# tohtsky/myFM

Measured on AMD Instinct MI355X. Metric: Gibbs iterations/sec (rank=32), higher is better.
Workload: dtype f64

## Files before the change

### include/myfm_hip.h

```cpp
#ifndef MYFM_HIP_H_
#define MYFM_HIP_H_

#include <stdint.h>

#ifdef __cplusplus
extern "C" {
#endif

#define MFM_OK 0
#define MFM_ERR_INVALID 1
#define MFM_ERR_RUNTIME 2
#define MFM_ERR_DEVICE 3

#define MFM_TASK_REGRESSION 0
#define MFM_TASK_CLASSIFICATION 1
#define MFM_TASK_ORDERED 2

typedef struct mfm_ctx mfm_ctx;
typedef struct mfm_design mfm_design;
typedef struct mfm_store mfm_store;

const char *mfm_version(void);
int mfm_device_count(void);
const char *mfm_global_error(void);
// ... 20 lines not shown
int mfm_peer_drop(mfm_ctx *ctx);
int mfm_set_main_levels(mfm_ctx *ctx, const int32_t *level, int64_t D0);
int mfm_set_row_offset(mfm_ctx *ctx, int64_t first_global_row);

int mfm_set_main(mfm_ctx *ctx, int64_t N, int64_t D0, const int64_t *indptr, const int32_t *indices,
                 const double *data, const double *y);
int mfm_add_block(mfm_ctx *ctx, int64_t B, int64_t Db, const int64_t *indptr, const int32_t *indices,
                  const double *data, const int64_t *original_to_block);
int mfm_set_groups(mfm_ctx *ctx, const int32_t *group_index, int64_t D, int32_t G);
int mfm_set_residual_policy(mfm_ctx *ctx, int32_t recomputable);
int mfm_finalize(mfm_ctx *ctx, int32_t rank);

int64_t mfm_dim_all(const mfm_ctx *ctx);
int mfm_plan_info(const mfm_ctx *ctx, int64_t *n_levels_main, int64_t *n_launches_per_sweep);
int mfm_plan_flags(const mfm_ctx *ctx);
#define MFM_RES_INFO_FIELDS 15
int mfm_res_info(const mfm_ctx *ctx, int64_t *out, int n_out, char *why, int why_len);
#define MFM_CELL_INFO_FIELDS 74
int mfm_cell_info(const mfm_ctx *ctx, int64_t *out, int n_out, char *why, int why_len);

int mfm_set_state(mfm_ctx *ctx, double w0, const double *w, const double *V);
int mfm_get_state(mfm_ctx *ctx, double *w0, double *w, double *V);
int mfm_set_w0(mfm_ctx *ctx, double w0);
int mfm_zero_w(mfm_ctx *ctx);
int mfm_get_e(mfm_ctx *ctx, double *e);
int mfm_get_q(mfm_ctx *ctx, double *q);
int mfm_set_e(mfm_ctx *ctx, const double *e);

int mfm_reduce_e(mfm_ctx *ctx, double *sum_e, double *sum_e2);
int mfm_shift_e(mfm_ctx *ctx, double delta);
int mfm_group_stats_w(mfm_ctx *ctx, const double *mu_w, double *sum, double *ssd);
// ... 193 lines not shown
```

### myfm_amd/_build.py

```python
import os
import subprocess
import sys
import sysconfig

HERE = os.path.dirname(os.path.abspath(__file__))
ROOT = os.path.dirname(HERE)
CSRC = os.path.join(HERE, "csrc")
INCLUDE = os.path.join(ROOT, "include")
HIP_LIB = os.path.join(HERE, "libmyfm_hip.so")
EXT_SUFFIX = sysconfig.get_config_var("EXT_SUFFIX") or ".so"
PYMOD = os.path.join(HERE, "_myfm" + EXT_SUFFIX)

HIP_UNITS = {
    "mfm_hip.hip": ["mfm_env.hpp", "mfm_common.hpp", "mfm_wave.hpp", "mfm_policies.hpp", "mfm_kernels.hpp", "mfm_mf_kernels.hpp", "mfm_res.hpp", "mfm_res_plan.hpp",
                    "mfm_plan.hpp", "mfm_block_kernels.hpp", "mfm_erfcx.hpp", "mfm_tasks.hpp", "mfm_tn.hpp", "mfm_philox.hpp", "mfm_predict.hpp", "mfm_samples.hpp", "mfm_dist.hpp", "mfm_rng.hpp", "mfm_mtjump.hpp", "mfm_cell.hpp",
                    "mfm_chain_api.hpp", "mfm_rng_state.hpp", "mfm_latent_api.hpp", "mfm_latent_host.hpp", "mfm_comm.hpp"],
    "mfm_latent.hip": ["mfm_env.hpp", "mfm_common.hpp", "mfm_rng_state.hpp", "mfm_latent_api.hpp"],
    "mfm_cell.hip": ["mfm_env.hpp", "mfm_common.hpp", "mfm_wave.hpp", "mfm_cell.hpp"],
    "mfm_chain.hip": ["mfm_env.hpp", "mfm_common.hpp", "mfm_wave.hpp", "mfm_policies.hpp", "mfm_chain_api.hpp", "mfm_chain_plan.hpp", "mfm_chain_stream.hpp"],
    "mfm_vb.hip": ["mfm_env.hpp", "mfm_common.hpp", "mfm_erfcx.hpp", "mfm_vb.hpp", "mfm_comm.hpp"],
    "mfm_pairs.hip": ["mfm_env.hpp", "mfm_common.hpp", "mfm_pairs.hpp", "mfm_pairs_rank.hpp", "mfm_pairs_ucb.hpp", "mfm_samples.hpp"],
    "mfm_foldin.hip": ["mfm_env.hpp", "mfm_common.hpp", "mfm_foldin.hpp", "mfm_foldin_handle.hpp", "mfm_philox.hpp", "mfm_samples.hpp"],
    "mfm_foldin_gibbs.hip": ["mfm_env.hpp", "mfm_common.hpp", "mfm_foldin.hpp", "mfm_foldin_gibbs.hpp", "mfm_foldin_gibbs_plan.hpp",
                             "mfm_foldin_handle.hpp", "mfm_tn.hpp", "mfm_philox.hpp", "mfm_samples.hpp"],
}
OBJ_DIR = os.path.join(CSRC, "_obj")
PYMOD_HEADERS = ["mfm_env.hpp", "mfm_hostnormals.hpp", "mfm_mtjump.hpp"]


# ... 83 lines not shown
```

### myfm_amd/_capi.py

```python
import ctypes as C
import os

import numpy as np
import scipy.sparse as sps

_HERE = os.path.dirname(os.path.abspath(__file__))
LIB_PATH = os.path.join(_HERE, "libmyfm_hip.so")

MFM_OK, MFM_ERR_INVALID, MFM_ERR_RUNTIME, MFM_ERR_DEVICE = 0, 1, 2, 3
TASK_REGRESSION, TASK_CLASSIFICATION, TASK_ORDERED = 0, 1, 2

SYMBOLS = [
    "mfm_version", "mfm_device_count", "mfm_global_error", "mfm_create", "mfm_destroy", "mfm_last_error",
    "mfm_set_stream", "mfm_synchronize", "mfm_set_main", "mfm_add_block", "mfm_set_groups", "mfm_finalize",
    "mfm_peer_info", "mfm_peer_set", "mfm_peer_model_info", "mfm_peer_set_model", "mfm_peer_export", "mfm_peer_import", "mfm_peer_drop", "mfm_set_residual_policy", "mfm_dim_all", "mfm_plan_info", "mfm_plan_flags", "mfm_res_info", "mfm_cell_info", "mfm_set_state", "mfm_get_state", "mfm_set_w0", "mfm_zero_w", "mfm_get_e",
    "mfm_get_q", "mfm_set_e", "mfm_reduce_e", "mfm_shift_e", "mfm_group_stats_w", "mfm_group_stats_V",
    "mfm_sweep_w", "mfm_sweep_V", "mfm_sweep_wV", "mfm_update_e_regression", "mfm_update_e_classification", "mfm_score_train",
    "mfm_oprobit_add_group", "mfm_oprobit_eval", "mfm_oprobit_sample_z", "mfm_hyper_stats", "mfm_timing_enable", "mfm_timing_select", "mfm_timing_reset",
    "mfm_timing_n_classes", "mfm_timing_class_name", "mfm_timing_get", "mfm_design_create", "mfm_design_add_block",
    "mfm_design_destroy", "mfm_design_last_error", "mfm_design_dim_all", "mfm_design_predict",
    "mfm_host_column_levels", "mfm_rng_prepare", "mfm_rng_seed_mt19937", "mfm_rng_set_program", "mfm_rng_prefetch", "mfm_rng_acquire",
    "mfm_rng_get_z", "mfm_design_score_ctx", "mfm_design_n_rows", "mfm_set_allreduce", "mfm_set_row_offset", "mfm_set_main_levels",
    "mfm_test_erfcx", "mfm_test_truncated_normal", "mfm_get_device", "mfm_set_shard", "mfm_comm_unique_id", "mfm_comm_init",
    "mfm_comm_stats", "mfm_comm_info", "mfm_store_create", "mfm_store_destroy", "mfm_store_last_error", "mfm_store_size", "mfm_store_push_ctx",
# ... 424 lines not shown
        self._ck(lib().mfm_rng_host_read(self.h, int(offset), int(n), _p(out)))
        return out[: int(n)]

    def rng_host_advance(self, words):
        self._ck(lib().mfm_rng_host_advance(self.h, int(words)))

    def set_residual_policy(self, recomputable):
        self._ck(lib().mfm_set_residual_policy(self.h, 1 if recomputable else 0))

    def plan_flags(self):
        f = lib().mfm_plan_flags(self.h)
        return {"qfree": bool(f & 1), "unit": bool(f & 2), "ell": bool(f & 4), "sharded": bool(f & 8), "soa": bool(f & 16),
                "fused_next": bool(f & 32), "sharded_fused": bool(f & 64), "mf": bool(f & 128), "resident": bool(f & 256), "cell": bool(f & 512), "streamed_chain": bool(f & 1024), "resident_overflow": bool(f & 2048)}

    RES_INFO = ("ready", "G", "RV", "RL", "RX", "umax", "n_items", "item_bits", "n_runs", "max_wg_users", "max_slice_items",
                "e_where", "n_rows", "s2_in_sweep_b", "lds_bytes")
    E_WHERE = ("rows", "slots", "slots_with_sums", "cell", "dropped")

    def res_info(self):
        out = np.zeros(len(self.RES_INFO), dtype=np.int64)
        why = C.create_string_buffer(256)
        self._ck(lib().mfm_res_info(self.h, _p(out), out.shape[0], why, len(why)))
        d = dict(zip(self.RES_INFO, (int(v) for v in out)))
        d["ready"] = bool(d["ready"])
        d["e_where"] = self.E_WHERE[d["e_where"]]
        d["why"] = why.value.decode()
        return d

    CELL_INFO = ("ready", "G", "umax", "item32", "n_streams", "n_fields", "N", "Npad", "max_steps", "chunk_max", "chunk_min",
                 "chunks_empty", "split_mask", "score_fb")
    CELL_STREAM_TYPE = ("U", "I", "C")
# ... 416 lines not shown
```

### myfm_amd/csrc/_myfm.cpp

```cpp
#include <thread>
#include <cstdio>
#include <pybind11/functional.h>
#include <pybind11/numpy.h>
#include <pybind11/pybind11.h>
#include <pybind11/stl.h>

#include <algorithm>
#include <cmath>
#include <chrono>
#include <cstdint>
#include <cstdlib>
#include <functional>
#include <limits>
#include <memory>
#include <random>
#include <set>
#include <sstream>
#include <stdexcept>
#include <string>
#include <tuple>
#include <type_traits>
#include <vector>

#include "mfm_env.hpp"
// ... 2880 lines not shown
             char path[512];
             if (mfm_comm_info(s.trainer->ctx, &n, path, sizeof(path)) != MFM_OK) throw std::runtime_error(mfm_global_error());
             return py::make_tuple((int)n, std::string(path));
           },
           "(ranks of the library's own RCCL communicator (ncclCommCount), path of the librccl.so it bound); (0, '') without one")
      .def("step", &GibbsSession::step, py::call_guard<py::gil_scoped_release>())
      .def("synchronize", &GibbsSession::synchronize)
      .def("residual", &GibbsSession::residual)
      .def("timing_enable", &GibbsSession::timing_enable)
      .def("timing_select", &GibbsSession::timing_select)
      .def("timing_reset", &GibbsSession::timing_reset)
      .def("timing", &GibbsSession::timing)
      .def("plan_info", &GibbsSession::plan_info)
      .def("latent_info", &GibbsSession::latent_info)
      .def("plan_flags", [](GibbsSession &s) { return mfm_plan_flags(s.trainer->ctx); })
      .def("peer_info",
           [](GibbsSession &s) {
             int32_t pending = 0;
             void *sum = nullptr, *flag = nullptr;
             int64_t sb = 0, fb = 0;
             ck(s.trainer->ctx, mfm_peer_info(s.trainer->ctx, &pending, &sum, &flag, &sb, &fb));
             return py::make_tuple(pending != 0, (uintptr_t)sum, (uintptr_t)flag, sb, fb);
           })
      .def("peer_set",
           [](GibbsSession &s, int world, int rank, const std::vector<uintptr_t> &sums, const std::vector<uintptr_t> &flags) {
             if ((int)sums.size() != world || (int)flags.size() != world) throw std::invalid_argument("peer_set: one buffer pair per rank");
             std::vector<void *> a, b;
             for (auto v : sums) a.push_back((void *)v);
             for (auto v : flags) b.push_back((void *)v);
             ck(s.trainer->ctx, mfm_peer_set(s.trainer->ctx, world, rank, a.data(), b.data()));
// ... 143 lines not shown
```

### myfm_amd/csrc/mfm_hip.hip

```cpp
#include <algorithm>
#include <cerrno>
#include <chrono>
#include <cmath>
#include <cstdio>
#include <cstring>
#include <map>
#include <memory>
#include <mutex>
#include <string>
#include <thread>
#include <type_traits>
#include <vector>

#include <fcntl.h>
#include <sys/file.h>
#include <sys/stat.h>
#include <unistd.h>

#include <hipcub/hipcub.hpp>

#include "mfm_common.hpp"
#include "mfm_kernels.hpp"
#include "mfm_plan.hpp"
#include "mfm_res_plan.hpp"
// ... 1561 lines not shown
    case VPath::ShardedTwoField: form = 64 | 128; break;
    case VPath::Deferred:
    case VPath::Generic:
    case VPath::Cell:
      break;
  }
  return (streamed ? 1024 : 0) | (ctx->res.ready && ctx->res.RX > 0 ? 2048 : 0) | form | (ctx->X.unit ? 2 : 0) | (ctx->X.ell_width >= 0 ? 4 : 0) |
         (ctx->comm.active() ? 8 : 0) | (ctx->res.ready ? 256 : 0) | (ctx->cell.ready ? 512 : 0);
}

int mfm_res_info(const mfm_ctx *ctx, int64_t *out, int n_out, char *why, int why_len) {
  if (!ctx || n_out < 0 || (n_out > 0 && !out) || why_len < 0 || (why_len > 0 && !why)) return MFM_ERR_INVALID;
  const ResPlan &rp = ctx->res;
  const int64_t v[MFM_RES_INFO_FIELDS] = {rp.ready ? 1 : 0, rp.G,       rp.RV,     rp.RL,           rp.RX,
                                          rp.umax,          rp.n_items, rp.item_bits, rp.n_runs,    rp.max_wg_users,
                                          rp.max_slice_items, (int64_t)ctx->e_where, rp.n_rows, rp.s2b, (int64_t)rp.lds_bytes};
  for (int i = 0; i < n_out; i++) out[i] = i < MFM_RES_INFO_FIELDS ? v[i] : 0;
  if (why_len > 0) {
    std::strncpy(why, rp.ready ? "" : rp.why.c_str(), (size_t)why_len - 1);
    why[why_len - 1] = 0;
  }
  return MFM_OK;
}

int mfm_cell_info(const mfm_ctx *ctx, int64_t *out, int n_out, char *why, int why_len) {
  if (!ctx || n_out < 0 || (n_out > 0 && !out) || why_len < 0 || (why_len > 0 && !why)) return MFM_ERR_INVALID;
  const CellPlan &cp = ctx->cell;
  int64_t v[MFM_CELL_INFO_FIELDS] = {0};
  const int m = (int)cp.fields.size(), ns = (int)cp.streams.size();
  int64_t split = 0;
  const bool typed = ns > 0 && cp.sU == 0;
// ... 915 lines not shown
```

### myfm_amd/csrc/mfm_res.hpp

```cpp
#pragma once
#include <algorithm>
#include <cstdlib>
#include <cstring>
#include <atomic>
#include <string>
#include <thread>
#include <type_traits>
#include <vector>

#include "mfm_common.hpp"
#include "mfm_mf_kernels.hpp"

namespace mfm {

#ifndef MFM_RES_CH
#define MFM_RES_CH 4
#endif
constexpr int RES_MAX_PEERS = 8;

struct ResArgs {
  double2 *eq;
  const double *e_in;
  double *e_slots;
  const int32_t *perm;
  const uint32_t *uidw;
  const uint32_t *headw;
  const int32_t *run_item;
  const int32_t *first_run;
  const int32_t *wg_run_ptr;
  const int32_t *wg_nruns;
  const int32_t *wg_user_ptr;
  const int2 *user_desc;
  const int32_t *wg_item_ptr;
  const int32_t *ent_ptr;
  const int2 *entries;
  const int32_t *scols;
  const int2 *item_desc;
  double *partials;
  double *dv;
  double *V;
  int64_t D;
  int f_begin, f_end;
  int linear;
  int n_sw;
  double *w;
  const double *zw;
  const double *lam_w, *mu_w;
  double e_shift;
  const double *z;
  const double *lam, *mu;
// ... 4 lines not shown
  int n_items, umax;
  unsigned long long *bar;
  int n_wg;
  int *error;
  unsigned long long *prof;
  int xworld, xrank;
  unsigned long long xepoch0;
  double *xsum[RES_MAX_PEERS];
  unsigned long long *xflag[RES_MAX_PEERS];
  unsigned long long *xarrive;
  int xmodel;
  double *xw[RES_MAX_PEERS], *xV[RES_MAX_PEERS];
  int ngx;
  int no_store;
  int xch_break;
};

__device__ __forceinline__ void res_store2(double *p, double a, double b) {
  __hip_atomic_store(p, a, __ATOMIC_RELAXED, __HIP_MEMORY_SCOPE_AGENT);
  __hip_atomic_store(p + 1, b, __ATOMIC_RELAXED, __HIP_MEMORY_SCOPE_AGENT);
}

enum { RES_BAR_START = 0, RES_BAR_TOP = 16, RES_BAR_XCNT = 32, RES_BAR_GEN = 160, RES_BAR_CENSUS = 288, RES_BAR_WORDS = 416 };
struct ResBar {
  int xcc;
  unsigned long long n_x, nx;
};

__device__ __forceinline__ bool res_spin(const ResArgs &a, const unsigned long long *w, unsigned long long target, bool &dead) {
  unsigned spins = 0;
// ... 125 lines not shown
#define RES_STAMP0(k) \
  if (a.prof && tid == 0) a.prof[(int64_t)g * a.n_sw * 64 + 56 + (k)] = __builtin_amdgcn_s_memrealtime()
  RES_STAMP0(0);
  if (tid == 0) res_bar_init(a, rbar, dead);
  RES_STAMP0(1);
  const int wv_hi = wv >> 2;
#define RES_PRIO(j)                  \
  if ((((j) & 1) ^ wv_hi) != 0)      \
    __builtin_amdgcn_s_setprio(1);   \
  else                               \
    __builtin_amdgcn_s_setprio(0)
  const int trash_run = a.wg_run_ptr[g] + a.wg_nruns[g];
#define RES_STAMP(k)                                                                                      \
  if (a.prof && tid == 0) a.prof[((int64_t)g * a.n_sw + (f - f_first)) * 64 + (k)] = __builtin_amdgcn_s_memrealtime()

  for (int i = tid; i < (S2B ? 3 : 2) * NW * U; i += NT) acc1[i] = 0.0;
  for (int i = tid; i < U; i += NT) utab[i] = d2_t{0.0, 0.0};

  res_u4_t uw[NG];
  unsigned ux[NG];
  unsigned hbv[NG], nbv[NG];
#pragma unroll
  for (int j = 0; j < NG; j++) {
    RES_GROUP_WORDS(a, NGt, j, uw[j], ux[j], hbv[j]);
    nbv[j] = hbv[j] | (j == 0 ? 1u : 0u);
  }
  const unsigned nbx0 = OVF && ngx > 0 ? a.headw[((int64_t)g * NGt + NG) * NT + tid] : 0u;
  double *eog = OVF ? a.e_slots + ((int64_t)g * Rt + 16 * NG) * NT + tid : nullptr;
  const uint32_t *uidw_x = a.uidw + ((int64_t)g * (5 * NGt) + 5 * NG) * NT + tid;
  const uint32_t *headw_x = a.headw + ((int64_t)g * NGt + NG) * NT + tid;
  const int run0 = a.first_run[g * NT + tid];
// ... 67 lines not shown
      }
    }
  }
  if (OVF) {
    for (int jx = 0; jx < ngx; jx++) {
#pragma unroll 4
      for (int i = 0; i < 16; i++) {
        const int64_t sl = 16 * (NG + jx) + i;
        const int row = a.e_in ? 0 : perm_g[sl * NT + tid];
        const double x = (a.e_in ? a.e_in[((int64_t)g * Rt + sl) * NT + tid] : a.eq[row < 0 ? 0 : row].x) + e_shift_k;
        eog[(16 * jx + i) * NT] = x;
      }
    }
  }
  __syncthreads();
  if (S2B) {
    const uint32_t *uidw_p = a.uidw + (int64_t)g * (5 * NGt) * NT + tid;
    const uint32_t *headw_p = a.headw + (int64_t)g * NGt * NT + tid;
    int run = run0 - 1;
    double c = 0.0;
#pragma unroll 1
    for (int jp = 0; jp < NGt; jp++) {
      const unsigned nb = headw_p[jp * NT] | (jp == 0 ? 1u : 0u);
      const unsigned uxp = uidw_p[(5 * jp + 4) * NT];
#pragma unroll 1
      for (int bb = 0; bb < 4; bb++) {
        const unsigned lo_ = uidw_p[(5 * jp + bb) * NT];
#pragma unroll 1
        for (int k = 0; k < B; k++) {
          if ((nb >> (4 * bb + k)) & 1u) {
            run++;
// ... 216 lines not shown
    const int wb = c0 + wv * per, we = wb + per < c1 ? wb + per : c1;
    const int i0 = a.wg_item_ptr[g], ni = a.wg_item_ptr[g + 1] - i0;
    const bool more = f + 1 < a.f_end;
    int ij = 0;
    double iold = 0.0, iz = 0.0, ivn = 0.0, ivq = 0.0, ilam = 0.0, imu = 0.0;
    if (tid < ni) {
      const int2 d = a.item_desc[i0 + tid];
      ij = d.x;
      iold = Vf[ij];
      iz = zf[ij];
      ivn = more ? a.V[(int64_t)(f + 1) * a.D + ij] : 0.0;
      if (S2B) ivq = f + 2 < a.f_end ? a.V[(int64_t)(f + 2) * a.D + ij] : 0.0;
      ilam = lamf[d.y];
      imu = muf[d.y];
    }
    int2 en[CH];
#pragma unroll
    for (int k = 0; k < CH; k++) en[k] = make_int2(0, 0);
    if (wb < we) {
#pragma unroll
      for (int k = 0; k < CH; k++) en[k] = a.entries[(int64_t)(wb + k < we ? wb + k : wb) * WAVE + lane];
    }
    res_grid_barrier(a, rbar, ++nbar, tid, dead);
    RES_STAMP(4);
    {
      const d2_t *part2 = (const d2_t *)a.partials;
      for (int cb = wb; cb < we; cb += CH) {
        d2_t sv[CH];
#pragma unroll
        for (int k = 0; k < CH; k++) sv[k] = part2[en[k].x];
        int il[CH];
#pragma unroll
        for (int k = 0; k < CH; k++) il[k] = en[k].y;
        if (cb + CH < we) {
#pragma unroll
          for (int k = 0; k < CH; k++) en[k] = a.entries[(int64_t)(cb + CH + k < we ? cb + CH + k : cb + CH) * WAVE + lane];
        }
#pragma unroll
        for (int k = 0; k < CH; k++) {
          if (cb + k >= we) break;
          __hip_atomic_fetch_add(&acc1[wv * U + il[k]], sv[k][0], __ATOMIC_RELAXED, __HIP_MEMORY_SCOPE_WORKGROUP);
          __hip_atomic_fetch_add(&acc2[wv * U + il[k]], sv[k][1], __ATOMIC_RELAXED, __HIP_MEMORY_SCOPE_WORKGROUP);
        }
      }
      __syncthreads();
      double S1 = 0.0, S2 = 0.0;
      if (tid < ni) {
#pragma unroll
        for (int w = 0; w < NW; w++) {
          S1 += acc1[w * U + tid];
          S2 += acc2[w * U + tid];
// ... 31 lines not shown
          }
        }
      }
      if (tid < ni) {
        const double fresh = PMainV::draw(S1, S2, iold, alpha_k, ilam, imu, iz);
        Vf[ij] = fresh;
        res_store2(a.dv + ((int64_t)(i0 + tid) << (DSH - 3)), fresh - iold, ivn);
        if (S2B) __hip_atomic_store(a.dv + 4 * (int64_t)(i0 + tid) + 2, ivq * ivq, __ATOMIC_RELAXED, __HIP_MEMORY_SCOPE_AGENT);
      }
    }
    RES_STAMP(5);
    res_grid_barrier(a, rbar, ++nbar, tid, dead);
    RES_STAMP(6);
  }
#undef RES_STAMP
  RES_STAMP0(3);
  if (!a.no_store) {
    int run_last = run0;
#pragma unroll
    for (int j = 0; j < NG; j++) {
#pragma unroll 1
      for (int bb = 0; bb < 4; bb++) {
        const unsigned h4 = (hbv[j] >> (4 * bb)) & 15u;
        int row[B], it[B];
#pragma unroll
        for (int k = 0; k < B; k++) {
          if (16 * j + 4 * bb + k > 0) run_last += (int)((h4 >> k) & 1u);
          it[k] = a.run_item[run_last];
          row[k] = perm_g[(16 * j + 4 * bb + k) * NT + tid];
        }
// ... 62 lines not shown
                              const double *__restrict__ theta2) {
  const int i = blockIdx.x * blockDim.x + threadIdx.x;
  if (blockIdx.x == 0)
    for (int k = threadIdx.x; k < RES_BAR_WORDS; k += blockDim.x) bar[k] = 0ull;
  if (i > n_items) return;
  const bool pad = i == n_items;
  dv[wd * i] = 0.0;
  dv[wd * i + 1] = pad ? 0.0 : theta ? theta[scols[i]] : 1.0;
  if (wd == 4) {
    const double c2 = !pad && theta2 ? theta2[scols[i]] : 0.0;
    dv[wd * i + 2] = c2 * c2;
    dv[wd * i + 3] = 0.0;
  }
}

__global__ void k_res_unpermute(const double *__restrict__ e_slots, const int32_t *__restrict__ perm, int64_t n_slots,
                                double2 *__restrict__ eq) {
  const int64_t i = (int64_t)blockIdx.x * blockDim.x + threadIdx.x;
  if (i >= n_slots) return;
  const int32_t row = perm[i];
  if (row >= 0) eq[row].x = e_slots[i];
}

struct ResScoreArgs {
  const uint32_t *uidw, *headw;
  const int32_t *first_run, *run_feat, *wg_user_ptr, *wg_fill;
  const int2 *user_desc;
  int umax, KS;
  const double *Vt, *w;
  double w0;
// ... 223 lines not shown
  int R() const { return RV + RL + RX; }
  bool allow_overflow = true;
  int64_t n_rows = 0, n_runs = 0;
  size_t lds_bytes = 0;
  int s2b = 0;
  int dv_doubles() const { return 1 << (res_dv_shift(s2b != 0) - 3); }
  bool plan_lds() {
    const size_t nw = (size_t)(NT / WAVE), lim = 160 * 1024 - 512;
    lds_bytes = (size_t)RL * NT * 8 + 2 * nw * umax * 8 + (size_t)umax * 16 + nw * 16 + nw * 4 + 64;
    if (lds_bytes > lim) return false;
    s2b = res_form(RV, RL, !allow_overflow, RX > 0, true) && lds_bytes + nw * umax * 8 <= lim ? 1 : 0;
    if (s2b) lds_bytes += nw * umax * 8;
    return true;
  }
  DevBuf<int32_t> perm, first_run, wg_run_ptr, wg_nruns, wg_user_ptr, wg_item_ptr, ent_ptr, scols;
  DevBuf<int2> entries;
  DevBuf<uint32_t> uidw, headw;
  DevBuf<int32_t> run_item;
  DevBuf<int2> user_desc, item_desc;
  DevBuf<double> partials, dv, e_slots;
  DevBuf<unsigned long long> bar;
  DevBuf<int32_t> run_feat, wg_fill;
  DevBuf<double> y_slots;
  DevBuf<double2> sums;
  int max_wg_users = 0, max_slice_items = 0;
  int xworld = 1, xrank = 0;
  bool peers_set = false;
  DevBuf<double> xsum;
  DevBuf<unsigned long long> xflag, xarrive;
  double *peer_sum[RES_MAX_PEERS] = {nullptr, nullptr, nullptr, nullptr, nullptr, nullptr, nullptr, nullptr};
  unsigned long long *peer_flag[RES_MAX_PEERS] = {nullptr, nullptr, nullptr, nullptr, nullptr, nullptr, nullptr, nullptr};
// ... 315 lines not shown
    h_uid = std::vector<uint16_t>();
    std::vector<int32_t> slice_of((size_t)n_items);
    for (int g = 0; g < G; g++)
      for (int c = h_iptr[g]; c < h_iptr[g + 1]; c++) slice_of[c] = g;
    std::vector<int32_t> h_eptr((size_t)G + 1, 0);
    {
      std::vector<int64_t> cnt((size_t)G, 0);
      for (int g = 0; g < G; g++)
        for (int32_t c : wg_run_item[g]) cnt[slice_of[c]]++;
      for (int g = 0; g < G; g++) {
        const int64_t e = h_eptr[g] + ((cnt[g] + WAVE - 1) / WAVE) * WAVE;
        if (e >= ((int64_t)1 << 31)) return fail("too many entries");
        h_eptr[g + 1] = (int32_t)e;
      }
    }
    std::vector<int2> h_entries((size_t)h_eptr[G], make_int2(zero_run, 0));
    {
      std::vector<int64_t> pos((size_t)G);
      for (int g = 0; g < G; g++) pos[g] = h_eptr[g];
      for (int g = 0; g < G; g++)
        for (size_t l = 0; l < wg_run_item[g].size(); l++) {
          const int32_t c = wg_run_item[g][l];
          const int sgl = slice_of[c];
          h_entries[(size_t)pos[sgl]++] = make_int2(run_base[g] + (int32_t)l, c - h_iptr[sgl]);
        }
    }
    if (h_entries.size() >= ((size_t)1 << 31)) return fail("too many entries");
    if (!plan_lds()) return fail("LDS");
    uidw.upload(h_uidw);
    headw.upload(h_headw);
    run_item.upload(h_run_item);
    perm.upload(h_perm);
    first_run.upload(h_first);
    wg_user_ptr.upload(h_uptr);
    user_desc.upload(h_udesc.data(), h_udesc.size());
    wg_item_ptr.upload(h_iptr);
    ent_ptr.upload(h_eptr);
    entries.upload(h_entries.data(), h_entries.size());
    wg_run_ptr.upload(run_base);
    wg_nruns.upload(nruns);
    e_slots.alloc((size_t)G * cap_slots);
    {
      std::vector<int32_t> h_run_feat(h_run_item.size() + 8, -1);
      for (size_t r = 0; r < h_run_item.size(); r++) h_run_feat[r] = h_run_item[r] < n_items ? items[(size_t)h_run_item[r]] : -1;
      run_feat.upload(h_run_feat);
      std::vector<int32_t> h_fill((size_t)G);
      for (int g = 0; g < G; g++) h_fill[g] = (int32_t)fill[g];
      wg_fill.upload(h_fill);
      sums.alloc((size_t)G);
      y_slots = DevBuf<double>();
    }
    h_nruns = nruns;
    if (env_flag("MFM_RES_PROF")) {
      h_diag.assign((size_t)G, "");
      for (int g = 0; g < G; g++) {
// ... 86 lines not shown
  a.w = w;
  a.zw = zw;
  a.lam_w = lam_w;
  a.mu_w = mu_w;
  a.e_shift = e_shift;
  a.perm = rp.perm.p;
  a.uidw = rp.uidw.p;
  a.headw = rp.headw.p;
  a.run_item = rp.run_item.p;
  a.first_run = rp.first_run.p;
  a.wg_user_ptr = rp.wg_user_ptr.p;
  a.user_desc = rp.user_desc.p;
  a.wg_item_ptr = rp.wg_item_ptr.p;
  a.ent_ptr = rp.ent_ptr.p;
  a.entries = rp.entries.p;
  a.wg_run_ptr = rp.wg_run_ptr.p;
  a.wg_nruns = rp.wg_nruns.p;
  a.scols = rp.scols.p;
  a.item_desc = rp.item_desc.p;
  a.partials = rp.partials.p;
  a.dv = rp.dv.p;
  a.V = V;
  a.D = D;
  a.f_begin = f_begin;
  a.f_end = f_end;
  a.z = zbase;
  a.lam = lam;
  a.mu = mu;
  a.group = group;
  a.n_groups = n_groups;
// ... 14 lines not shown
    a.xsum[r] = rp.peer_sum[r];
    a.xflag[r] = rp.peer_flag[r];
    a.xw[r] = rp.peer_w[r];
    a.xV[r] = rp.peer_V[r];
  }
  if (xch && !rp.peers_set) throw Error(MFM_ERR_RUNTIME, "row-sharded persistent sweep: the peers' exchange buffers are not set (mfm_peer_set)");
  static int prof_launch = 0;
  const bool prof = env_flag("MFM_RES_PROF") && ++prof_launch == env_int("MFM_RES_PROF", 0);
  DevBuf<unsigned long long> prof_buf;
  if (prof) {
    prof_buf.alloc((size_t)rp.G * a.n_sw * 64);
    MFM_HIP_CHECK(hipMemsetAsync(prof_buf.p, 0, (size_t)rp.G * a.n_sw * 512, s));
    a.prof = prof_buf.p;
  }
  const int K = a.n_sw;
  double bytes = (8.0 + (load_slots ? 0.0 : 4.0) + 1.4 + (no_store ? 0.0 : 8.0)) * rp.n_rows + K * 48.0 * rp.n_runs;
  if (rp.RX) bytes += (double)K * (16.0 + 1.75) * (double)rp.G * rp.NT * rp.RX;
  {
    const int f_second = f_begin + (w ? 0 : 1);
    hipLaunchKernelGGL(k_res_init_dv, dim3((rp.n_items + 256) / 256), dim3(256), 0, s,
                       w ? (const double *)nullptr : V + (int64_t)f_begin * D, rp.scols.p, rp.n_items,
                       rp.dv.p, rp.bar.p, rp.dv_doubles(), rp.s2b && f_second < f_end ? V + (int64_t)f_second * D : (const double *)nullptr);
  }
  TimedLaunch t(tm, s, kernel_class, bytes);
  res_launch(res_kernel(rp, xch), rp.G, rp.lds_bytes, s, a);
  MFM_HIP_CHECK(hipGetLastError());
  if (xch) rp.xepoch += (unsigned long long)a.n_sw;
  if (prof) {
    MFM_HIP_CHECK(hipStreamSynchronize(s));
    const int K2 = a.n_sw;
    std::vector<unsigned long long> h((size_t)rp.G * K2 * 64);
// ... 159 lines not shown
```

### myfm_amd/csrc/mfm_res_plan.hpp

```cpp
#pragma once
#include <chrono>

#include <hipcub/hipcub.hpp>

#include "mfm_res.hpp"

namespace mfm {

namespace rp {

constexpr int TB = 256;

__global__ void k_rows(const int32_t *__restrict__ colidx, int64_t N, int32_t *__restrict__ bflag, int32_t *__restrict__ ucnt,
                       int32_t *__restrict__ icnt, int32_t *__restrict__ red) {
  const int64_t r = (int64_t)blockIdx.x * blockDim.x + threadIdx.x;
  int32_t mu = -1, mi = 0x7fffffff;
  if (r < N) {
    const int2 c = ((const int2 *)colidx)[r];
    const bool b = r == 0 || c.x != colidx[2 * (r - 1)];
    bflag[r] = b ? 1 : 0;
    if (b) atomicAdd(&ucnt[c.x], 1);
    atomicAdd(&icnt[c.y], 1);
    mu = c.x;
    mi = c.y;
// ... 86 lines not shown
  perm[(int64_t)g * cap + (int64_t)rr * NT + t] = row;
  uid[(int64_t)g * cap + sidx] = (uint16_t)(uord1[row] - 1 - ucut[g]);
  headf[p] = (sidx == 0 || k != key[p - 1]) ? 1 : 0;
}

__global__ void k_wg_runs(const int32_t *__restrict__ hs, const int32_t *__restrict__ rowcut, int G, int32_t *__restrict__ hrun0) {
  const int g = blockIdx.x * blockDim.x + threadIdx.x;
  if (g > G) return;
  hrun0[g] = rowcut[g] > 0 ? hs[rowcut[g] - 1] : 0;
}

__global__ void k_fill32(int32_t *p, int64_t n, int32_t v) {
  const int64_t i = (int64_t)blockIdx.x * blockDim.x + threadIdx.x;
  if (i < n) p[i] = v;
}
__global__ void k_fill_int2(int2 *p, int64_t n, int2 v) {
  const int64_t i = (int64_t)blockIdx.x * blockDim.x + threadIdx.x;
  if (i < n) p[i] = v;
}

__global__ void k_runs(const uint32_t *__restrict__ key, const int32_t *__restrict__ headf, const int32_t *__restrict__ hs,
                       const int32_t *__restrict__ hrun0, const int32_t *__restrict__ run_base, int item_bits, int64_t N,
                       int32_t *__restrict__ run_item_c, int32_t *__restrict__ run_item, int32_t *__restrict__ runs_per_item) {
  const int64_t p = (int64_t)blockIdx.x * blockDim.x + threadIdx.x;
  if (p >= N || !headf[p]) return;
  const uint32_t k = key[p];
  const int g = (int)(k >> item_bits);
  const int32_t item = (int32_t)(k & ((1u << item_bits) - 1u));
  const int32_t kc = hs[p] - 1;
  run_item_c[kc] = item;
  run_item[run_base[g] + kc - hrun0[g]] = item;
  atomicAdd(&runs_per_item[item], 1);
}
// ... 72 lines not shown
}

__global__ void k_slice_keys(const int32_t *__restrict__ run_item_c, const int32_t *__restrict__ iptr, int G, int64_t n, uint32_t *__restrict__ key,
                             int32_t *__restrict__ val) {
  __shared__ int32_t cut[1026];
  for (int i = threadIdx.x; i <= G; i += blockDim.x) cut[i] = iptr[i];
  __syncthreads();
  const int64_t k = (int64_t)blockIdx.x * blockDim.x + threadIdx.x;
  if (k >= n) return;
  key[k] = (uint32_t)upper_group(cut, G, run_item_c[k]);
  val[k] = (int32_t)k;
}

__global__ void k_entries(const uint32_t *__restrict__ key, const int32_t *__restrict__ val, const int32_t *__restrict__ run_item_c,
                          const int32_t *__restrict__ hrun0, const int32_t *__restrict__ run_base, const int32_t *__restrict__ iptr,
                          const int32_t *__restrict__ eptr, const int32_t *__restrict__ sstart, int G, int64_t n, int2 *__restrict__ entries) {
  __shared__ int32_t cut[1026];
  for (int i = threadIdx.x; i <= G; i += blockDim.x) cut[i] = hrun0[i];
  __syncthreads();
  const int64_t q = (int64_t)blockIdx.x * blockDim.x + threadIdx.x;
  if (q >= n) return;
  const int sl = (int)key[q];
  const int32_t kc = val[q];
  const int g = upper_group(cut, G, kc);
  entries[eptr[sl] + (q - sstart[sl])] = make_int2(run_base[g] + (kc - cut[g]), run_item_c[kc] - iptr[sl]);
}

template <class T>
static inline std::vector<T> download(const T *p, size_t n, hipStream_t s) {
  std::vector<T> h(n);
  if (n) MFM_HIP_CHECK(hipMemcpyAsync(h.data(), p, n * sizeof(T), hipMemcpyDeviceToHost, s));
  MFM_HIP_CHECK(hipStreamSynchronize(s));
  return h;
}

static inline void inclusive_sum(const int32_t *in, int32_t *out, int64_t n, DevBuf<char> &tmp, hipStream_t s) {
  size_t bytes = 0;
  MFM_HIP_CHECK(hipcub::DeviceScan::InclusiveSum(nullptr, bytes, in, out, (int)n, s));
  if (tmp.n < bytes) tmp.alloc(bytes);
  MFM_HIP_CHECK(hipcub::DeviceScan::InclusiveSum(tmp.p, bytes, in, out, (int)n, s));
// ... 174 lines not shown
  if (rpn.umax > 1024) return rpn.fail("internal: user field");
  const int UW = 5 * (R / 16), HW = R / 16;
  rpn.uidw.alloc((size_t)G * UW * NT);
  rpn.headw.alloc((size_t)G * HW * NT);
  hipLaunchKernelGGL(k_pack, grid((int64_t)G * HW * NT), dim3(TB), 0, s, uid.p, headf.p, rowcut.p, G, R, NT, rpn.umax, rpn.uidw.p, rpn.headw.p);
  std::vector<int32_t> h_eptr((size_t)G + 1, 0), h_sstart((size_t)G + 1, 0);
  for (int g = 0; g < G; g++) {
    const int64_t cnt = h_slot_ptr[h_iptr[g + 1]] - h_slot_ptr[h_iptr[g]];
    const int64_t e = h_eptr[g] + ((cnt + WAVE - 1) / WAVE) * WAVE;
    if (e >= ((int64_t)1 << 31)) return rpn.fail("too many entries");
    h_eptr[g + 1] = (int32_t)e;
    h_sstart[g + 1] = h_sstart[g] + (int32_t)cnt;
  }
  rpn.wg_item_ptr.upload(h_iptr);
  rpn.ent_ptr.upload(h_eptr);
  rpn.entries.alloc((size_t)h_eptr[G]);
  if (h_eptr[G]) hipLaunchKernelGGL(k_fill_int2, grid(h_eptr[G]), dim3(TB), 0, s, rpn.entries.p, (int64_t)h_eptr[G], make_int2(zero_run, 0));
  if (counter > 0) {
    DevBuf<int32_t> sstart;
    sstart.upload(h_sstart);
    DevBuf<uint32_t> sk, sk2;
    DevBuf<int32_t> sv, sv2;
    sk.alloc((size_t)counter);
    sk2.alloc((size_t)counter);
    sv.alloc((size_t)counter);
    sv2.alloc((size_t)counter);
    hipLaunchKernelGGL(k_slice_keys, grid(counter), dim3(TB), 0, s, run_item_c.p, rpn.wg_item_ptr.p, G, counter, sk.p, sv.p);
    sort_pairs(sk, sk2, sv, sv2, counter, gbits, tmp, s);
    hipLaunchKernelGGL(k_entries, grid(counter), dim3(TB), 0, s, sk2.p, sv2.p, run_item_c.p, hrun0.p, rpn.wg_run_ptr.p, rpn.wg_item_ptr.p,
                       rpn.ent_ptr.p, sstart.p, G, counter, rpn.entries.p);
    MFM_HIP_CHECK(hipStreamSynchronize(s));
  }
  lap("slices, pack, entries");
  DevBuf<int32_t> d_group;
  if (group_of && (int64_t)group_of->size() >= D0) d_group.upload(group_of->data(), (size_t)D0);
  rpn.user_desc.alloc((size_t)h_uptr[G]);
  hipLaunchKernelGGL(k_user_desc, grid((int64_t)n_users + n_emp), dim3(TB), 0, s, d_users.p, empties.p, d_ucut.p, rpn.wg_user_ptr.p, d_group.p, G,
                     n_users, n_emp, rpn.user_desc.p);
  rpn.item_desc.alloc((size_t)n_items);
  hipLaunchKernelGGL(k_item_desc, grid(n_items), dim3(TB), 0, s, rpn.scols.p, d_group.p, n_items, rpn.item_desc.p);
  rpn.run_feat.alloc((size_t)zero_run + 1 + 8);
  hipLaunchKernelGGL(k_run_feat, grid((int64_t)zero_run + 9), dim3(TB), 0, s, rpn.run_item.p, rpn.scols.p, n_items, (int64_t)zero_run + 1,
                     (int64_t)zero_run + 9, rpn.run_feat.p);
  {
    std::vector<int32_t> h_fill((size_t)G);
    for (int g = 0; g < G; g++) h_fill[g] = h_rowcut[g + 1] - h_rowcut[g];
    rpn.wg_fill.upload(h_fill);
  }
  if (!rpn.plan_lds()) return rpn.fail("LDS");
  rpn.e_slots.alloc((size_t)G * cap_slots);
  rpn.sums.alloc((size_t)G);
  rpn.y_slots = DevBuf<double>();
  rpn.h_nruns = nruns;
  rpn.h_diag.clear();
  rpn.partials.alloc((size_t)2 * ((size_t)zero_run + 1));
  MFM_HIP_CHECK(hipMemsetAsync(rpn.partials.p, 0, (size_t)16 * ((size_t)zero_run + 1), s));
  rpn.dv.alloc((size_t)rpn.dv_doubles() * (n_items + 1));
  rpn.bar.alloc(RES_BAR_WORDS);
  MFM_HIP_CHECK(hipStreamSynchronize(s));
  MFM_HIP_CHECK(hipGetLastError());
  lap("descriptors, buffers");
  rpn.ready = true;
  rpn.why.clear();
  return true;
}

static inline std::string res_plan_compare(const ResPlan &a, const ResPlan &b, hipStream_t s) {
  if (a.G != b.G || a.RV != b.RV || a.RL != b.RL || a.RX != b.RX || a.umax != b.umax || a.item_bits != b.item_bits || a.n_items != b.n_items ||
      a.n_rows != b.n_rows || a.n_runs != b.n_runs || a.lds_bytes != b.lds_bytes || a.s2b != b.s2b || a.max_wg_users != b.max_wg_users ||
      a.max_slice_items != b.max_slice_items)
    return "scalars";
  auto same = [&](const void *p, size_t np, const void *q, size_t nq, size_t elem) {
    if (np != nq) return false;
    std::vector<char> x(np * elem), y(nq * elem);
    if (np) {
      MFM_HIP_CHECK(hipMemcpyAsync(x.data(), p, np * elem, hipMemcpyDeviceToHost, s));
      MFM_HIP_CHECK(hipMemcpyAsync(y.data(), q, nq * elem, hipMemcpyDeviceToHost, s));
    }
    MFM_HIP_CHECK(hipStreamSynchronize(s));
    return x == y;
  };
#define MFM_RP_CMP(f) \
  if (!same(a.f.p, a.f.n, b.f.p, b.f.n, sizeof(*a.f.p))) return #f;
  MFM_RP_CMP(perm)
  MFM_RP_CMP(first_run)
  MFM_RP_CMP(wg_run_ptr)
  MFM_RP_CMP(wg_nruns)
  MFM_RP_CMP(wg_user_ptr)
  MFM_RP_CMP(wg_item_ptr)
  MFM_RP_CMP(ent_ptr)
  MFM_RP_CMP(scols)
  MFM_RP_CMP(entries)
  MFM_RP_CMP(uidw)
  MFM_RP_CMP(headw)
  MFM_RP_CMP(run_item)
  MFM_RP_CMP(user_desc)
  MFM_RP_CMP(item_desc)
  MFM_RP_CMP(run_feat)
  MFM_RP_CMP(wg_fill)
#undef MFM_RP_CMP
  return "";
}

}
```

Baseline: 377.3.

## Pack resident entries into 32-bit words and precompute per-group s2 count table

Per-slice (run, item) entries shrink from int2 to one packed 32-bit word: 23 bits of run index and 9 bits of item offset. The packed form is used only when runs fit and the plan is not row-sharded. This cuts the bytes each sweep reads while streaming entries. A new plan-time kernel also precomputes the per-wave user counts that the s2 statistic needs, so the resident sweep loads a table instead of re-walking the uidw/headw bitmaps each time. The cost is extra decode ALU in the inner loop and a fixed 9-bit item field, which would corrupt results if a slice ever held more than 511 items.

```diff
diff --git a/include/myfm_hip.h b/include/myfm_hip.h
--- a/include/myfm_hip.h
+++ b/include/myfm_hip.h
@@ -58,7 +58,7 @@
 int64_t mfm_dim_all(const mfm_ctx *ctx);
 int mfm_plan_info(const mfm_ctx *ctx, int64_t *n_levels_main, int64_t *n_launches_per_sweep);
 int mfm_plan_flags(const mfm_ctx *ctx);
-#define MFM_RES_INFO_FIELDS 15
+#define MFM_RES_INFO_FIELDS 16
 int mfm_res_info(const mfm_ctx *ctx, int64_t *out, int n_out, char *why, int why_len);
 #define MFM_CELL_INFO_FIELDS 74
 int mfm_cell_info(const mfm_ctx *ctx, int64_t *out, int n_out, char *why, int why_len);
diff --git a/myfm_amd/_build.py b/myfm_amd/_build.py
--- a/myfm_amd/_build.py
+++ b/myfm_amd/_build.py
@@ -12,7 +12,7 @@
 PYMOD = os.path.join(HERE, "_myfm" + EXT_SUFFIX)
 
 HIP_UNITS = {
-    "mfm_hip.hip": ["mfm_env.hpp", "mfm_common.hpp", "mfm_wave.hpp", "mfm_policies.hpp", "mfm_kernels.hpp", "mfm_mf_kernels.hpp", "mfm_res.hpp", "mfm_res_plan.hpp",
+    "mfm_hip.hip": ["mfm_env.hpp", "mfm_common.hpp", "mfm_wave.hpp", "mfm_policies.hpp", "mfm_kernels.hpp", "mfm_mf_kernels.hpp", "mfm_res.hpp", "mfm_res_entry.hpp", "mfm_res_plan.hpp",
                     "mfm_plan.hpp", "mfm_block_kernels.hpp", "mfm_erfcx.hpp", "mfm_tasks.hpp", "mfm_tn.hpp", "mfm_philox.hpp", "mfm_predict.hpp", "mfm_samples.hpp", "mfm_dist.hpp", "mfm_rng.hpp", "mfm_mtjump.hpp", "mfm_cell.hpp",
                     "mfm_chain_api.hpp", "mfm_rng_state.hpp", "mfm_latent_api.hpp", "mfm_latent_host.hpp", "mfm_comm.hpp"],
     "mfm_latent.hip": ["mfm_env.hpp", "mfm_common.hpp", "mfm_rng_state.hpp", "mfm_latent_api.hpp"],
diff --git a/myfm_amd/_capi.py b/myfm_amd/_capi.py
--- a/myfm_amd/_capi.py
+++ b/myfm_amd/_capi.py
@@ -462,7 +462,7 @@
                 "fused_next": bool(f & 32), "sharded_fused": bool(f & 64), "mf": bool(f & 128), "resident": bool(f & 256), "cell": bool(f & 512), "streamed_chain": bool(f & 1024), "resident_overflow": bool(f & 2048)}
 
     RES_INFO = ("ready", "G", "RV", "RL", "RX", "umax", "n_items", "item_bits", "n_runs", "max_wg_users", "max_slice_items",
-                "e_where", "n_rows", "s2_in_sweep_b", "lds_bytes")
+                "e_where", "n_rows", "s2_in_sweep_b", "lds_bytes", "entry_bytes")
     E_WHERE = ("rows", "slots", "slots_with_sums", "cell", "dropped")
 
     def res_info(self):
diff --git a/myfm_amd/csrc/_myfm.cpp b/myfm_amd/csrc/_myfm.cpp
--- a/myfm_amd/csrc/_myfm.cpp
+++ b/myfm_amd/csrc/_myfm.cpp
@@ -2918,6 +2918,13 @@
       .def("plan_info", &GibbsSession::plan_info)
       .def("latent_info", &GibbsSession::latent_info)
       .def("plan_flags", [](GibbsSession &s) { return mfm_plan_flags(s.trainer->ctx); })
+      .def("res_info",
+           [](GibbsSession &s) {
+             std::vector<int64_t> v(MFM_RES_INFO_FIELDS, 0);
+             ck(s.trainer->ctx, mfm_res_info(s.trainer->ctx, v.data(), (int)v.size(), nullptr, 0));
+             return v;
+           },
+           "the persistent sweep's layout: the MFM_RES_INFO_FIELDS values of mfm_res_info (myfm_hip.h)")
       .def("peer_info",
            [](GibbsSession &s) {
              int32_t pending = 0;
diff --git a/myfm_amd/csrc/mfm_hip.hip b/myfm_amd/csrc/mfm_hip.hip
--- a/myfm_amd/csrc/mfm_hip.hip
+++ b/myfm_amd/csrc/mfm_hip.hip
@@ -1599,7 +1599,8 @@
   const ResPlan &rp = ctx->res;
   const int64_t v[MFM_RES_INFO_FIELDS] = {rp.ready ? 1 : 0, rp.G,       rp.RV,     rp.RL,           rp.RX,
                                           rp.umax,          rp.n_items, rp.item_bits, rp.n_runs,    rp.max_wg_users,
-                                          rp.max_slice_items, (int64_t)ctx->e_where, rp.n_rows, rp.s2b, (int64_t)rp.lds_bytes};
+                                          rp.max_slice_items, (int64_t)ctx->e_where, rp.n_rows, rp.s2b, (int64_t)rp.lds_bytes,
+                                          rp.ent_bytes};
   for (int i = 0; i < n_out; i++) out[i] = i < MFM_RES_INFO_FIELDS ? v[i] : 0;
   if (why_len > 0) {
     std::strncpy(why, rp.ready ? "" : rp.why.c_str(), (size_t)why_len - 1);
diff --git a/myfm_amd/csrc/mfm_res.hpp b/myfm_amd/csrc/mfm_res.hpp
--- a/myfm_amd/csrc/mfm_res.hpp
+++ b/myfm_amd/csrc/mfm_res.hpp
@@ -10,6 +10,7 @@
 
 #include "mfm_common.hpp"
 #include "mfm_mf_kernels.hpp"
+#include "mfm_res_entry.hpp"
 
 namespace mfm {
 
@@ -33,7 +34,7 @@
   const int2 *user_desc;
   const int32_t *wg_item_ptr;
   const int32_t *ent_ptr;
-  const int2 *entries;
+  const uint32_t *entries;
   const int32_t *scols;
   const int2 *item_desc;
   double *partials;
@@ -68,6 +69,8 @@
   int ngx;
   int no_store;
   int xch_break;
+  int ent4;
+  const double *s2_lin;
 };
 
 __device__ __forceinline__ void res_store2(double *p, double a, double b) {
@@ -223,7 +226,10 @@
 #define RES_STAMP(k)                                                                                      \
   if (a.prof && tid == 0) a.prof[((int64_t)g * a.n_sw + (f - f_first)) * 64 + (k)] = __builtin_amdgcn_s_memrealtime()
 
-  for (int i = tid; i < (S2B ? 3 : 2) * NW * U; i += NT) acc1[i] = 0.0;
+  const bool s2_tab = S2B && a.s2_lin != nullptr;
+  for (int i = tid; i < (S2B && !s2_tab ? 3 : 2) * NW * U; i += NT) acc1[i] = 0.0;
+  if (s2_tab)
+    for (int i = tid; i < NW * U; i += NT) acc3[i] = a.s2_lin[(int64_t)g * (NW * U) + i];
   for (int i = tid; i < U; i += NT) utab[i] = d2_t{0.0, 0.0};
 
   res_u4_t uw[NG];
@@ -321,7 +327,7 @@
     }
   }
   __syncthreads();
-  if (S2B) {
+  if (S2B && !s2_tab) {
     const uint32_t *uidw_p = a.uidw + (int64_t)g * (5 * NGt) * NT + tid;
     const uint32_t *headw_p = a.headw + (int64_t)g * NGt * NT + tid;
     int run = run0 - 1;
@@ -568,12 +574,22 @@
       ilam = lamf[d.y];
       imu = muf[d.y];
     }
+    const bool ent4 = a.ent4 != 0;
+#define RES_ENTRIES(c_)                                                                                                    \
+  if (ent4) {                                                                                                              \
+    _Pragma("unroll") for (int k = 0; k < CH; k++)                                                                         \
+      en[k] = make_int2((int)a.entries[(int64_t)((c_) + k < we ? (c_) + k : (c_)) * WAVE + lane], 0);                      \
+  } else {                                                                                                                 \
+    _Pragma("unroll") for (int k = 0; k < CH; k++)                                                                         \
+      en[k] = ((const int2 *)a.entries)[(int64_t)((c_) + k < we ? (c_) + k : (c_)) * WAVE + lane];                         \
+  }
+#define RES_ENT_RUN(e_) (ent4 ? res_entry_run((uint32_t)(e_).x) : (e_).x)
+#define RES_ENT_ITEM(e_) (ent4 ? res_entry_item((uint32_t)(e_).x) : (e_).y)
     int2 en[CH];
 #pragma unroll
     for (int k = 0; k < CH; k++) en[k] = make_int2(0, 0);
     if (wb < we) {
-#pragma unroll
-      for (int k = 0; k < CH; k++) en[k] = a.entries[(int64_t)(wb + k < we ? wb + k : wb) * WAVE + lane];
+      RES_ENTRIES(wb);
     }
     res_grid_barrier(a, rbar, ++nbar, tid, dead);
     RES_STAMP(4);
@@ -582,13 +598,12 @@
       for (int cb = wb; cb < we; cb += CH) {
         d2_t sv[CH];
 #pragma unroll
-        for (int k = 0; k < CH; k++) sv[k] = part2[en[k].x];
+        for (int k = 0; k < CH; k++) sv[k] = part2[RES_ENT_RUN(en[k])];
         int il[CH];
 #pragma unroll
-        for (int k = 0; k < CH; k++) il[k] = en[k].y;
+        for (int k = 0; k < CH; k++) il[k] = RES_ENT_ITEM(en[k]);
         if (cb + CH < we) {
-#pragma unroll
-          for (int k = 0; k < CH; k++) en[k] = a.entries[(int64_t)(cb + CH + k < we ? cb + CH + k : cb + CH) * WAVE + lane];
+          RES_ENTRIES(cb + CH);
         }
 #pragma unroll
         for (int k = 0; k < CH; k++) {
@@ -650,6 +665,9 @@
     RES_STAMP(6);
   }
 #undef RES_STAMP
+#undef RES_ENTRIES
+#undef RES_ENT_RUN
+#undef RES_ENT_ITEM
   RES_STAMP0(3);
   if (!a.no_store) {
     int run_last = run0;
@@ -742,6 +760,36 @@
   }
 }
 
+__global__ __launch_bounds__(512) void k_res_s2_lin(const uint32_t *__restrict__ uidw, const uint32_t *__restrict__ headw,
+                                                    const int32_t *__restrict__ run_item, const int32_t *__restrict__ first_run,
+                                                    int NGt, int umax, int n_items, double *__restrict__ s2_lin) {
+  extern __shared__ unsigned res_s2_cnt[];
+  constexpr int NT = 512, NW = NT / WAVE;
+  const int g = (int)blockIdx.x, tid = threadIdx.x, wv = tid >> 6;
+  for (int i = tid; i < NW * umax; i += NT) res_s2_cnt[i] = 0u;
+  __syncthreads();
+  const uint32_t *uidw_p = uidw + (int64_t)g * (5 * NGt) * NT + tid;
+  const uint32_t *headw_p = headw + (int64_t)g * NGt * NT + tid;
+  int run = first_run[g * NT + tid] - 1;
+  bool real = false;
+  for (int jp = 0; jp < NGt; jp++) {
+    const unsigned nb = headw_p[jp * NT] | (jp == 0 ? 1u : 0u);
+    const unsigned uxp = uidw_p[(5 * jp + 4) * NT];
+    for (int bb = 0; bb < 4; bb++) {
+      const unsigned lo_ = uidw_p[(5 * jp + bb) * NT];
+      for (int k = 0; k < 4; k++) {
+        if ((nb >> (4 * bb + k)) & 1u) {
+          run++;
+          real = run_item[run] < n_items;
+        }
+        if (real) atomicAdd(&res_s2_cnt[wv * umax + RES_UID(lo_, uxp, bb, k)], 1u);
+      }
+    }
+  }
+  __syncthreads();
+  for (int i = tid; i < NW * umax; i += NT) s2_lin[(int64_t)g * (NW * umax) + i] = (double)res_s2_cnt[i];
+}
+
 __global__ void k_res_unpermute(const double *__restrict__ e_slots, const int32_t *__restrict__ perm, int64_t n_slots,
                                 double2 *__restrict__ eq) {
   const int64_t i = (int64_t)blockIdx.x * blockDim.x + threadIdx.x;
@@ -995,7 +1043,20 @@
     return true;
   }
   DevBuf<int32_t> perm, first_run, wg_run_ptr, wg_nruns, wg_user_ptr, wg_item_ptr, ent_ptr, scols;
-  DevBuf<int2> entries;
+  DevBuf<uint32_t> entries;
+  int ent_bytes = 8;
+  void choose_entry_width(int64_t zero_run) { ent_bytes = res_entry_bytes(zero_run, !allow_overflow); }
+  DevBuf<double> s2_lin;
+  void fill_s2_lin(hipStream_t s) {
+    s2_lin = DevBuf<double>();
+    if (!s2b) return;
+    const size_t nw = (size_t)(NT / WAVE);
+    s2_lin.alloc((size_t)G * nw * umax);
+    hipLaunchKernelGGL(k_res_s2_lin, dim3(G), dim3(NT), nw * umax * sizeof(unsigned), s, uidw.p, headw.p, run_item.p, first_run.p,
+                       R() / 16, umax, n_items, s2_lin.p);
+    MFM_HIP_CHECK(hipGetLastError());
+    MFM_HIP_CHECK(hipStreamSynchronize(s));
+  }
   DevBuf<uint32_t> uidw, headw;
   DevBuf<int32_t> run_item;
   DevBuf<int2> user_desc, item_desc;
@@ -1341,7 +1402,18 @@
         h_eptr[g + 1] = (int32_t)e;
       }
     }
-    std::vector<int2> h_entries((size_t)h_eptr[G], make_int2(zero_run, 0));
+    choose_entry_width(zero_run);
+    const size_t ew = (size_t)ent_bytes / 4;
+    std::vector<uint32_t> h_entries(ew * (size_t)h_eptr[G]);
+    auto put_entry = [&](size_t i, int32_t run, int32_t item) {
+      if (ew == 1) {
+        h_entries[i] = res_entry_pack(run, item);
+      } else {
+        h_entries[2 * i] = (uint32_t)run;
+        h_entries[2 * i + 1] = (uint32_t)item;
+      }
+    };
+    for (size_t i = 0; i < (size_t)h_eptr[G]; i++) put_entry(i, zero_run, 0);
     {
       std::vector<int64_t> pos((size_t)G);
       for (int g = 0; g < G; g++) pos[g] = h_eptr[g];
@@ -1349,10 +1421,10 @@
         for (size_t l = 0; l < wg_run_item[g].size(); l++) {
           const int32_t c = wg_run_item[g][l];
           const int sgl = slice_of[c];
-          h_entries[(size_t)pos[sgl]++] = make_int2(run_base[g] + (int32_t)l, c - h_iptr[sgl]);
-        }
-    }
-    if (h_entries.size() >= ((size_t)1 << 31)) return fail("too many entries");
+          put_entry((size_t)pos[sgl]++, run_base[g] + (int32_t)l, c - h_iptr[sgl]);
+        }
+    }
+    if ((size_t)h_eptr[G] >= ((size_t)1 << 31)) return fail("too many entries");
     if (!plan_lds()) return fail("LDS");
     uidw.upload(h_uidw);
     headw.upload(h_headw);
@@ -1363,9 +1435,10 @@
     user_desc.upload(h_udesc.data(), h_udesc.size());
     wg_item_ptr.upload(h_iptr);
     ent_ptr.upload(h_eptr);
-    entries.upload(h_entries.data(), h_entries.size());
+    entries.upload(h_entries);
     wg_run_ptr.upload(run_base);
     wg_nruns.upload(nruns);
+    fill_s2_lin(nullptr);
     e_slots.alloc((size_t)G * cap_slots);
     {
       std::vector<int32_t> h_run_feat(h_run_item.size() + 8, -1);
@@ -1482,6 +1555,8 @@
   a.wg_item_ptr = rp.wg_item_ptr.p;
   a.ent_ptr = rp.ent_ptr.p;
   a.entries = rp.entries.p;
+  a.ent4 = rp.ent_bytes == 4 ? 1 : 0;
+  a.s2_lin = rp.s2b && w ? rp.s2_lin.p : nullptr;
   a.wg_run_ptr = rp.wg_run_ptr.p;
   a.wg_nruns = rp.wg_nruns.p;
   a.scols = rp.scols.p;
@@ -1526,7 +1601,7 @@
     a.prof = prof_buf.p;
   }
   const int K = a.n_sw;
-  double bytes = (8.0 + (load_slots ? 0.0 : 4.0) + 1.4 + (no_store ? 0.0 : 8.0)) * rp.n_rows + K * 48.0 * rp.n_runs;
+  double bytes = (8.0 + (load_slots ? 0.0 : 4.0) + 1.4 + (no_store ? 0.0 : 8.0)) * rp.n_rows + K * (40.0 + rp.ent_bytes) * rp.n_runs;
   if (rp.RX) bytes += (double)K * (16.0 + 1.75) * (double)rp.G * rp.NT * rp.RX;
   {
     const int f_second = f_begin + (w ? 0 : 1);
diff --git a/myfm_amd/csrc/mfm_res_entry.hpp b/myfm_amd/csrc/mfm_res_entry.hpp
--- /dev/null
+++ b/myfm_amd/csrc/mfm_res_entry.hpp
@@ -0,0 +1,23 @@
+#pragma once
+#include <cstdint>
+
+#if defined(__HIPCC__)
+#define MFM_RES_ENTRY_FN __host__ __device__ inline
+#else
+#define MFM_RES_ENTRY_FN inline
+#endif
+
+namespace mfm {
+
+constexpr int RES_ENT_ITEM_BITS = 9, RES_ENT_RUN_BITS = 32 - RES_ENT_ITEM_BITS;
+
+MFM_RES_ENTRY_FN int res_entry_bytes(int64_t max_run, bool row_sharded) {
+  return !row_sharded && max_run >= 0 && max_run < ((int64_t)1 << RES_ENT_RUN_BITS) ? 4 : 8;
+}
+MFM_RES_ENTRY_FN uint32_t res_entry_pack(int32_t run, int32_t item) {
+  return ((uint32_t)run << RES_ENT_ITEM_BITS) | (uint32_t)item;
+}
+MFM_RES_ENTRY_FN int32_t res_entry_run(uint32_t w) { return (int32_t)(w >> RES_ENT_ITEM_BITS); }
+MFM_RES_ENTRY_FN int32_t res_entry_item(uint32_t w) { return (int32_t)(w & ((1u << RES_ENT_ITEM_BITS) - 1u)); }
+
+}
diff --git a/myfm_amd/csrc/mfm_res_plan.hpp b/myfm_amd/csrc/mfm_res_plan.hpp
--- a/myfm_amd/csrc/mfm_res_plan.hpp
+++ b/myfm_amd/csrc/mfm_res_plan.hpp
@@ -124,9 +124,13 @@
   const int64_t i = (int64_t)blockIdx.x * blockDim.x + threadIdx.x;
   if (i < n) p[i] = v;
 }
-__global__ void k_fill_int2(int2 *p, int64_t n, int2 v) {
+__global__ void k_fill_entries(uint32_t *p, int64_t n, int32_t run, int32_t item, bool ent4) {
   const int64_t i = (int64_t)blockIdx.x * blockDim.x + threadIdx.x;
-  if (i < n) p[i] = v;
+  if (i >= n) return;
+  if (ent4)
+    p[i] = res_entry_pack(run, item);
+  else
+    ((int2 *)p)[i] = make_int2(run, item);
 }
 
 __global__ void k_runs(const uint32_t *__restrict__ key, const int32_t *__restrict__ headf, const int32_t *__restrict__ hs,
@@ -229,7 +233,8 @@
 
 __global__ void k_entries(const uint32_t *__restrict__ key, const int32_t *__restrict__ val, const int32_t *__restrict__ run_item_c,
                           const int32_t *__restrict__ hrun0, const int32_t *__restrict__ run_base, const int32_t *__restrict__ iptr,
-                          const int32_t *__restrict__ eptr, const int32_t *__restrict__ sstart, int G, int64_t n, int2 *__restrict__ entries) {
+                          const int32_t *__restrict__ eptr, const int32_t *__restrict__ sstart, int G, int64_t n, uint32_t *__restrict__ entries,
+                          bool ent4) {
   __shared__ int32_t cut[1026];
   for (int i = threadIdx.x; i <= G; i += blockDim.x) cut[i] = hrun0[i];
   __syncthreads();
@@ -238,7 +243,12 @@
   const int sl = (int)key[q];
   const int32_t kc = val[q];
   const int g = upper_group(cut, G, kc);
-  entries[eptr[sl] + (q - sstart[sl])] = make_int2(run_base[g] + (kc - cut[g]), run_item_c[kc] - iptr[sl]);
+  const int64_t at = eptr[sl] + (q - sstart[sl]);
+  const int32_t run = run_base[g] + (kc - cut[g]), item = run_item_c[kc] - iptr[sl];
+  if (ent4)
+    entries[at] = res_entry_pack(run, item);
+  else
+    ((int2 *)entries)[at] = make_int2(run, item);
 }
 
 template <class T>
@@ -443,8 +453,10 @@
   }
   rpn.wg_item_ptr.upload(h_iptr);
   rpn.ent_ptr.upload(h_eptr);
-  rpn.entries.alloc((size_t)h_eptr[G]);
-  if (h_eptr[G]) hipLaunchKernelGGL(k_fill_int2, grid(h_eptr[G]), dim3(TB), 0, s, rpn.entries.p, (int64_t)h_eptr[G], make_int2(zero_run, 0));
+  rpn.choose_entry_width(zero_run);
+  const bool ent4 = rpn.ent_bytes == 4;
+  rpn.entries.alloc((size_t)(rpn.ent_bytes / 4) * (size_t)h_eptr[G]);
+  if (h_eptr[G]) hipLaunchKernelGGL(k_fill_entries, grid(h_eptr[G]), dim3(TB), 0, s, rpn.entries.p, (int64_t)h_eptr[G], zero_run, 0, ent4);
   if (counter > 0) {
     DevBuf<int32_t> sstart;
     sstart.upload(h_sstart);
@@ -457,7 +469,7 @@
     hipLaunchKernelGGL(k_slice_keys, grid(counter), dim3(TB), 0, s, run_item_c.p, rpn.wg_item_ptr.p, G, counter, sk.p, sv.p);
     sort_pairs(sk, sk2, sv, sv2, counter, gbits, tmp, s);
     hipLaunchKernelGGL(k_entries, grid(counter), dim3(TB), 0, s, sk2.p, sv2.p, run_item_c.p, hrun0.p, rpn.wg_run_ptr.p, rpn.wg_item_ptr.p,
-                       rpn.ent_ptr.p, sstart.p, G, counter, rpn.entries.p);
+                       rpn.ent_ptr.p, sstart.p, G, counter, rpn.entries.p, ent4);
     MFM_HIP_CHECK(hipStreamSynchronize(s));
   }
   lap("slices, pack, entries");
@@ -477,6 +489,7 @@
     rpn.wg_fill.upload(h_fill);
   }
   if (!rpn.plan_lds()) return rpn.fail("LDS");
+  rpn.fill_s2_lin(s);
   rpn.e_slots.alloc((size_t)G * cap_slots);
   rpn.sums.alloc((size_t)G);
   rpn.y_slots = DevBuf<double>();
@@ -497,7 +510,7 @@
 static inline std::string res_plan_compare(const ResPlan &a, const ResPlan &b, hipStream_t s) {
   if (a.G != b.G || a.RV != b.RV || a.RL != b.RL || a.RX != b.RX || a.umax != b.umax || a.item_bits != b.item_bits || a.n_items != b.n_items ||
       a.n_rows != b.n_rows || a.n_runs != b.n_runs || a.lds_bytes != b.lds_bytes || a.s2b != b.s2b || a.max_wg_users != b.max_wg_users ||
-      a.max_slice_items != b.max_slice_items)
+      a.max_slice_items != b.max_slice_items || a.ent_bytes != b.ent_bytes)
     return "scalars";
   auto same = [&](const void *p, size_t np, const void *q, size_t nq, size_t elem) {
     if (np != nq) return false;
@@ -527,6 +540,7 @@
   MFM_RP_CMP(item_desc)
   MFM_RP_CMP(run_feat)
   MFM_RP_CMP(wg_fill)
+  MFM_RP_CMP(s2_lin)
 #undef MFM_RP_CMP
   return "";
 }
```

Measured after the change: 382.3, median of 6. +1.3%, better.
